# florianwechsung/alfi

Measured on AMD Instinct MI355X. Metric: V-cycles/sec on ldc3d P2-P0 (DoF*smooths/sec in dof_smooths_per_s), higher is better.
Workload: dtype f64

## Files before the change

alfi_amd/csrc/cond_layout.h:

```cpp
#pragma once
#include <cstdint>

#ifdef __HIPCC__
#define ALFI_HD __host__ __device__
#else
#define ALFI_HD
#endif

struct CondChunk {
  int64_t off;
  int64_t ubase;
  int64_t sidx0;
  int64_t stage_off;
  int32_t xq0, xq1;
  int32_t bq0, bq1;
  int32_t e0, ne;
  int32_t u0, nu;
  int32_t nI;
  int32_t xp0, bp0;
  int32_t pad;
};

#ifndef ALFI_COND_SIGMA_ROWS
#define ALFI_COND_SIGMA_ROWS 64
#endif
constexpr int COND_SIGMA_ROWS = ALFI_COND_SIGMA_ROWS;

constexpr int64_t COND_PER_PATCH_MIN = 1024;

ALFI_HD inline int cond_patch_waves(int max_pairs) {
#ifdef ALFI_COND_WAVES_FORCE
  (void)max_pairs;
  return ALFI_COND_WAVES_FORCE;
#else
  return max_pairs <= 64 ? 1 : max_pairs <= 128 ? 2 : max_pairs <= 256 ? 4 : 8;
#endif
}

ALFI_HD inline int cond_ldim(int rows) { return (rows + 1) & ~1; }
ALFI_HD inline int cond_pairs(int rows) { return (rows + 1) / 2; }
ALFI_HD inline int64_t cond_group_doubles(int m, int sc) {
  return (int64_t)cond_ldim(m) * m + (int64_t)cond_ldim(sc) * m + (int64_t)cond_ldim(m) * sc;
}
```

alfi_amd/csrc/kernels_bigpatch.hip:

```cpp
#include <algorithm>
#include <cstdlib>
#include <vector>
#include "common.h"
#include "row_piece.h"
#include "cond_apply.h"

constexpr int BIG_NB = 64;
constexpr int BIG_MAX_NP = PATCH_MAX;

template <int BS>
__global__ __launch_bounds__(256) void big_gather_kernel(int64_t p0, const int32_t* __restrict__ rowptr,
                                                          const int32_t* __restrict__ colidx,
                                                          const double* __restrict__ vals, int flat,
                                                          const int64_t* __restrict__ patch_ptr,
                                                          const int32_t* __restrict__ patch_dofs,
                                                          const int64_t* __restrict__ scr_ptr, double* __restrict__ scr) {
  __shared__ int32_t dofs_s[BIG_MAX_NP];
  const int64_t p = p0 + blockIdx.y;
  const int64_t off = patch_ptr[p];
  const int n = (int)(patch_ptr[p + 1] - off);
  const int N = (n + BIG_NB - 1) / BIG_NB * BIG_NB;
  double* S = scr + scr_ptr[blockIdx.y];
  for (int i = threadIdx.x; i < n; i += 256) dofs_s[i] = patch_dofs[off + i];
  const int chunk = (N + gridDim.x - 1) / gridDim.x;
// ... 683 lines not shown
  for (int k = 0; k < m; ++k) {
    double v = (lane >= k && lane < m) ? fabs(A[lane * m + k]) : -1.0;
    if (!(v == v)) v = INFINITY;
    int idx = lane;
#pragma unroll
    for (int o = 32; o > 0; o >>= 1) {
      const double ov = __shfl_xor(v, o);
      const int oi = __shfl_xor(idx, o);
      if (ov > v || (ov == v && oi < idx)) { v = ov; idx = oi; }
    }
    if (!(v > 0.0) || v == INFINITY) { bad = true; break; }
    if (lane == 0) perm[k] = idx;
    if (idx != k && lane < m) {
      const double t = A[k * m + lane];
      A[k * m + lane] = A[idx * m + lane];
      A[idx * m + lane] = t;
    }
    __syncthreads();
    const double ip = 1.0 / A[k * m + k];
    if (lane > k && lane < m) {
      const double l = A[lane * m + k] * ip;
      A[lane * m + k] = l;
      for (int j = k + 1; j < m; ++j) A[lane * m + j] = __builtin_fma(-l, A[k * m + j], A[lane * m + j]);
    }
    __syncthreads();
  }
  if (bad) {
    if (lane == 0) atomicExch(status, 1);
    return;
  }
  auto solve = [&](double* B, int nrhs, bool identity) {
    const bool act = lane < nrhs;
    for (int i = 0; i < m; ++i) Y[i * 64 + lane] = act ? (identity ? (i == lane ? 1.0 : 0.0) : B[(int64_t)lane * ldm + i]) : 0.0;
    for (int k = 0; k < m; ++k) {
      const int pk = perm[k];
      if (pk != k) {
        const double t = Y[k * 64 + lane];
        Y[k * 64 + lane] = Y[pk * 64 + lane];
        Y[pk * 64 + lane] = t;
      }
    }
    for (int i = 1; i < m; ++i) {
      double acc = Y[i * 64 + lane];
      for (int j = 0; j < i; ++j) acc = __builtin_fma(-A[i * m + j], Y[j * 64 + lane], acc);
      Y[i * 64 + lane] = acc;
    }
    for (int i = m - 1; i >= 0; --i) {
      double acc = Y[i * 64 + lane];
      for (int j = i + 1; j < m; ++j) acc = __builtin_fma(-A[i * m + j], Y[j * 64 + lane], acc);
      Y[i * 64 + lane] = acc / A[i * m + i];
    }
    if (act)
      for (int i = 0; i < m; ++i) B[(int64_t)lane * ldm + i] = Y[i * 64 + lane];
  };
  solve(W, sc, false);
  solve(X, m, true);
}

__global__ __launch_bounds__(256) void cond_schur_kernel(int64_t p0, CondDev cd, const int64_t* __restrict__ patch_ptr,
                                                          const int64_t* __restrict__ scr_ptr, double* __restrict__ scr) {
  const int64_t p = p0 + blockIdx.x;
  const int n = (int)(patch_ptr[p + 1] - patch_ptr[p]);
  const int s = n - cd.p_nI[p];
  const int N = (s + BIG_NB - 1) / BIG_NB * BIG_NB;
  double* S = scr + scr_ptr[blockIdx.x];
  for (int64_t g = cd.gptr[p]; g < cd.gptr[p + 1]; ++g) {
    const int m = cd.g_m[g], sc = cd.g_sc[g];
    const int ldm = cond_ldim(m), ldsc = cond_ldim(sc);
    const double* B = cd.mat + cd.g_mat[g] + (int64_t)ldm * m;
    const double* W = B + (int64_t)ldsc * m;
    const int32_t* si = cd.sidx + cd.g_sidx[g];
    for (int e = threadIdx.x; e < sc * sc; e += 256) {
      const int i = e % sc, j = e / sc;
      double acc = 0.0;
      for (int k = 0; k < m; ++k) acc = __builtin_fma(B[(int64_t)k * ldsc + i], W[(int64_t)j * ldm + k], acc);
      S[(int64_t)si[i] * N + si[j]] -= acc;
    }
    __syncthreads();
  }
}



template <bool NT, int COND_WAVES, int RU>
__global__ __launch_bounds__(64 * COND_WAVES) void cond_front_kernel(int64_t p0, int64_t p1, CondDev cd,
                                                                     const int64_t* __restrict__ patch_ptr,
                                                                     const int64_t* __restrict__ stage_ptr,
                                                                     const double* __restrict__ x, double* __restrict__ stage,
                                                                     int ordered) {
  extern __shared__ double cond_dsmem[];
  constexpr int NT_ = 64 * COND_WAVES;
  if (p0 + blockIdx.x >= p1) return;
  const int64_t p = ordered ? cd.order[blockIdx.x] : p0 + blockIdx.x;
  const int64_t off = patch_ptr[p];
  const int n = (int)(patch_ptr[p + 1] - off);
  const int nI = cd.p_nI[p];
  const int s = n - nI;
  const int64_t uo0 = cd.uptr[p];
  double* xs = cond_dsmem;
  double* ts = xs + n;
  double* us = ts + nI;
  for (int i0 = threadIdx.x; i0 < n; i0 += 4 * NT_) {
    int32_t d[4];
#pragma unroll
    for (int u = 0; u < 4; ++u) d[u] = (i0 + u * NT_ < n) ? cd.dofs[off + i0 + u * NT_] : 0;
    double v[4];
#pragma unroll
    for (int u = 0; u < 4; ++u) v[u] = (i0 + u * NT_ < n) ? x[d[u]] : 0.0;
#pragma unroll
    for (int u = 0; u < 4; ++u)
      if (i0 + u * NT_ < n) xs[i0 + u * NT_] = v[u];
  }
  __syncthreads();
  double* tmp = cd.tmp + off;
  const int64_t xp0 = cd.xp_ptr[p], bp0 = cd.bp_ptr[p];
  const int nxp = (int)(cd.xp_ptr[p + 1] - xp0), nbp = (int)(cd.bp_ptr[p + 1] - bp0);
  for (int q0 = 0; q0 < nxp; q0 += NT_) {
    const int q = q0 + threadIdx.x;
    const bool act = q < nxp;
    const int32_t g = act ? cd.xp_grp[xp0 + q] : (int32_t)cd.gptr[p];
    const int m = cd.g_m[g], o = cd.g_off[g], i = 2 * (q - cd.g_xp[g]);
    double t0 = 0.0, t1 = 0.0;
    cond_row2_dot<NT, RU>(cd.mat + cd.g_mat[g] + i, cond_ldim(m), act ? m : 0, xs + o, t0, t1);
    if (act) {
      ts[o + i] = t0;
      tmp[o + i] = t0;
      if (i + 1 < m) {
        ts[o + i + 1] = t1;
        tmp[o + i + 1] = t1;
      }
    }
  }
  __syncthreads();
  for (int q0 = 0; q0 < nbp; q0 += NT_) {
    const int q = q0 + threadIdx.x;
    const bool act = q < nbp;
    const int32_t g = act ? cd.bp_grp[bp0 + q] : (int32_t)cd.gptr[p];
    const int m = cd.g_m[g], sc = cd.g_sc[g], j = 2 * (q - cd.g_bp[g]);
    const int64_t ue = uo0 + cd.g_uoff[g] + j;
    const int32_t d0 = act ? cd.u_dst[ue] : 0, d1 = (act && j + 1 < sc) ? cd.u_dst[ue + 1] : 0;
    double u0 = 0.0, u1 = 0.0;
    cond_row2_dot<NT, RU>(cd.mat + cd.g_mat[g] + (int64_t)cond_ldim(m) * m + j, cond_ldim(sc), act ? m : 0,
                          ts + cd.g_off[g], u0, u1);
    if (act) {
      us[d0] = u0;
      if (j + 1 < sc) us[d1] = u1;
    }
  }
  __syncthreads();
  const int64_t srow0 = cd.sptr[p];
  const int32_t qb = cd.s_uptr[srow0];
  double* rhs = stage + stage_ptr[p] + nI;
  for (int i = threadIdx.x; i < s; i += NT_) {
    double acc = xs[nI + i];
    const int32_t qe = cd.s_uptr[srow0 + i + 1] - qb;
    for (int32_t q = cd.s_uptr[srow0 + i] - qb; q < qe; ++q) acc -= us[q];
    rhs[i] = acc;
  }
}

template <bool NT>
__global__ __launch_bounds__(256) void cond_sigma_kernel(int64_t c0, CondDev cd, const int64_t* __restrict__ patch_ptr,
                                                         const int64_t* __restrict__ stage_ptr,
                                                         const double* __restrict__ stage) {
  extern __shared__ double cond_dsmem[];
  const int64_t c = c0 + blockIdx.x;
  const int64_t p = cd.ch_patch[c];
  const int r0 = cd.ch_row[c];
  const int64_t off = patch_ptr[p];
  const int n = (int)(patch_ptr[p + 1] - off);
  const int nI = cd.p_nI[p];
  const int s = n - nI;
  const int ld = (s + 1) & ~1;
  const double* rhs = stage + stage_ptr[p] + nI;
  const int r1 = min(ld, r0 + COND_SIGMA_ROWS);
  const int share = (((r1 - r0) + 3) / 4 + 15) & ~15;
// ... 451 lines not shown
      hipLaunchKernelGGL(big_store_kernel, dim3(sx, (unsigned)nb), block, 0, ctx->stream, p0, d_patch_ptr, d_inv_ptr,
                         d_scr_ptr, result, inv);
    }
    e = hipGetLastError();
    if (e != hipSuccess) break;
  }
  if (e == hipSuccess) e = hipStreamSynchronize(ctx->stream);
  if (e != hipSuccess) return alfi_set_error(ctx, ALFI_E_HIP, "large-block factorisation failed: %s", hipGetErrorString(e));
  return 0;
}

int launch_big_factor_range(alfi_level* L, double* inv, int64_t p0, int64_t p1) {
  BigSource src;
  src.L = L;
  return big_factor_core(L->ctx, src, p0, p1, L->lay.patch_ptr.data(), L->patch_ptr, L->inv_ptr, inv, L->status);
}

int launch_big_factor_transfer(alfi_transfer* T) {
  BigSource src;
  src.T = T;
  std::vector<int64_t> hptr(T->nblk + 1);
  for (int64_t b = 0; b <= T->nblk; ++b) hptr[b] = b * T->m;
  return big_factor_core(T->ctx, src, 0, T->nblk, hptr.data(), T->pm_ptr, T->pm_inv_ptr, T->binv, T->status);
}

int launch_coarse_factor(alfi_level* L, double* out) {
  alfi_ctx* ctx = L->ctx;
  BigSource src;
  src.C = L;
  const int64_t hptr[2] = {0, L->n};
  int64_t* dptr = nullptr;
  ALFI_HIP_CHECK(ctx, hipMalloc((void**)&dptr, sizeof(hptr)));
  hipError_t e = hipMemcpy(dptr, hptr, sizeof(hptr), hipMemcpyHostToDevice);
  int rc = e == hipSuccess ? big_factor_core(ctx, src, 0, 1, hptr, dptr, nullptr, nullptr, L->status, out)
                           : alfi_set_error(ctx, ALFI_E_HIP, "hipMemcpy: %s", hipGetErrorString(e));
  (void)hipFree(dptr);
  if (rc == 0 && ctx->big_arena_bytes > ((size_t)1 << 30)) {
    (void)hipFree(ctx->big_arena);
    ctx->big_arena = nullptr;
    ctx->big_arena_bytes = 0;
  }
  return rc;
}

int launch_cond_factor(alfi_level* L) {
  BigSource src;
  src.K = L;
  return big_factor_core(L->ctx, src, 0, L->npatch, L->cplan.sptr.data(), L->cd.sptr, L->cd.sinv_ptr, L->cd.sinv, L->status);
}

int launch_cond_schur_one(alfi_level* L, int64_t p, const int64_t* d_zero, double* scr) {
  BigSource src;
  src.K = L;
  src.pivot_groups = true;
  src.fill(L->ctx, p, 1, d_zero, scr);
  ALFI_HIP_CHECK(L->ctx, hipGetLastError());
  return 0;
}

int launch_cond_apply_range(alfi_level* L, int64_t p0, int64_t p1, const double* x) {
  alfi_ctx* ctx = L->ctx;
  if (p1 <= p0) return 0;
  if (!L->cd.tmp) return alfi_set_error(ctx, ALFI_E_STATE, "condensed apply without its scratch (alfi_patches_set_groups)");
  dim3 grid((unsigned)(p1 - p0));
  const int ordered = p0 == 0 && p1 == L->npatch && L->cd.order ? 1 : 0;
  const int64_t c0 = L->cplan.chptr[p0], c1 = L->cplan.chptr[p1];
  if (p1 - p0 < COND_PER_PATCH_MIN) {
    const int64_t k0 = L->cplan.gcptr[p0], k1 = L->cplan.gcptr[p1];
    const size_t lds_f = (size_t)L->cplan.lds_gfront, lds_b = (size_t)L->cplan.lds_gback;
    const size_t lds_s = (size_t)(L->cplan.max_s + 2 + COND_SIGMA_ROWS) * sizeof(double);
    if (k1 > k0)
      hipLaunchKernelGGL((cond_gfront_kernel<false>), dim3((unsigned)(k1 - k0)), dim3(256), lds_f, ctx->stream, k0, L->cd, x);
    if (c1 > c0)
      hipLaunchKernelGGL((cond_gsigma_kernel<true>), dim3((unsigned)(c1 - c0)), dim3(256), lds_s, ctx->stream, c0, L->cd,
                         L->patch_ptr, L->stage_ptr, x, L->stage);
    if (k1 > k0)
      hipLaunchKernelGGL((cond_gback_kernel<false>), dim3((unsigned)(k1 - k0)), dim3(256), lds_b, ctx->stream, k0, L->cd,
                         L->stage);
    ALFI_HIP_CHECK(ctx, hipGetLastError());
    return 0;
  }
  const size_t lds_f = (size_t)L->cplan.lds_front, lds_s = (size_t)(L->cplan.max_s + 2) * sizeof(double);
  const size_t lds_b = (size_t)L->cplan.lds_back;
#define ALFI_COND_LAUNCH3(WV)                                                                                             \
  do {                                                                                                                    \
    if (lds_f > 64 * 1024)                                                                                                \
      ALFI_HIP_CHECK(ctx, hipFuncSetAttribute(reinterpret_cast<const void*>(&cond_front_kernel<false, WV, 8>),            \
                                              hipFuncAttributeMaxDynamicSharedMemorySize, (int)lds_f));                   \
    hipLaunchKernelGGL((cond_front_kernel<false, WV, 8>), dim3(grid.x), dim3(64 * WV), lds_f, ctx->stream, p0, p1, L->cd, \
                       L->patch_ptr, L->stage_ptr, x, L->stage, ordered);                                                 \
    if (c1 > c0)                                                                                                          \
      hipLaunchKernelGGL((cond_sigma_kernel<true>), dim3((unsigned)(c1 - c0)), dim3(256), lds_s, ctx->stream, c0, L->cd,  \
                         L->patch_ptr, L->stage_ptr, L->stage);                                                           \
    if (lds_b > 64 * 1024)                                                                                                \
      ALFI_HIP_CHECK(ctx, hipFuncSetAttribute(reinterpret_cast<const void*>(&cond_back_kernel<false, WV, 8>),             \
                                              hipFuncAttributeMaxDynamicSharedMemorySize, (int)lds_b));                   \
    hipLaunchKernelGGL((cond_back_kernel<false, WV, 8>), dim3(grid.x), dim3(64 * WV), lds_b, ctx->stream, p0, p1, L->cd,  \
                       L->patch_ptr, L->stage_ptr, L->stage, ordered);                                                    \
  } while (0)
#ifdef ALFI_COND_WAVES_FORCE
  ALFI_COND_LAUNCH3(ALFI_COND_WAVES_FORCE);
#else
  switch (cond_patch_waves(L->cplan.max_pairs)) {
    case 1: ALFI_COND_LAUNCH3(1); break;
    case 2: ALFI_COND_LAUNCH3(2); break;
    case 4: ALFI_COND_LAUNCH3(4); break;
    default: ALFI_COND_LAUNCH3(8); break;
  }
#endif
#undef ALFI_COND_LAUNCH3
  ALFI_HIP_CHECK(ctx, hipGetLastError());
  return 0;
}

#include "mf_coarse.h"
```

alfi_amd/csrc/patch_plan.h:

```cpp
#pragma once
#include <algorithm>
#include <climits>
#include <cstdarg>
#include <cstdint>
#include <cstdio>
#include <string>
#include <vector>
#include "cond_layout.h"

#pragma GCC visibility push(hidden)

constexpr int PLAN_E_ARG = -2;
constexpr int SMALL_PATCH_MAX = 160;
constexpr int PATCH_MAX = 4096;
constexpr int COND_LDS_MAX_BYTES = 150 * 1024;
constexpr int COND_GROUP_MAX = 64;
constexpr int COND_CHUNK_PAIRS = 256;
constexpr int MULT_WAVE_NODES = 64;

inline int plan_fail(std::string* err, const char* fmt, ...) {
  char buf[1024];
  va_list ap;
  va_start(ap, fmt);
  vsnprintf(buf, sizeof(buf), fmt, ap);
// ... 67 lines not shown
  out->stage_ptr = std::move(stage_ptr);
  out->dof_ptr = std::move(dof_ptr);
  out->dof_pos = std::move(dof_pos);
  out->sum_n = sum_n;
  out->sum_n2 = sum_n2;
  out->max_np = max_np;
  out->inv_doubles = ip;
  out->stage_len = sp;
  return 0;
}

ALFI_HD inline int64_t piece_index(int r, int c, int n, int ld, int min_rows) {
  int row0 = r & ~127, rows = 128;
  if (row0 + 128 > ld) {
    const int rem = ld - row0;
    int rr = r - row0;
    for (int bit = 64; bit >= min_rows; bit >>= 1) {
      if (rem & bit) {
        if (rr < bit) {
          rows = bit;
          break;
        }
        rr -= bit;
        row0 += bit;
      }
    }
  }
  return (int64_t)row0 * n + (int64_t)c * rows + (r - row0);
}
ALFI_HD inline int64_t patch_inv_index(int r, int c, int n, int ld) { return piece_index(r, c, n, ld, 2); }

constexpr int F32_ROWS = 4;
constexpr int F32_ALIGN = 32;

ALFI_HD inline int f32_ld(int n) { return (n + F32_ROWS - 1) & ~(F32_ROWS - 1); }
ALFI_HD inline int64_t f32_patch_floats(int n) { return ((int64_t)n * f32_ld(n) + F32_ALIGN - 1) & ~(int64_t)(F32_ALIGN - 1); }
ALFI_HD inline int64_t f32_inv_index(int r, int c, int n) { return piece_index(r, c, n, f32_ld(n), F32_ROWS); }
inline int64_t plan_f32_offsets(int64_t npatch, const int64_t* pptr, std::vector<int64_t>* f32_ptr) {
  f32_ptr->resize((size_t)npatch + 1);
  int64_t ip = 0;
  for (int64_t p = 0; p < npatch; ++p) {
    (*f32_ptr)[(size_t)p] = ip;
    ip += f32_patch_floats((int)(pptr[p + 1] - pptr[p]));
  }
  (*f32_ptr)[(size_t)npatch] = ip;
  return ip;
}
inline int64_t plan_f32_ranges(int64_t npatch, const int64_t* inv_ptr, int64_t cap, std::vector<int64_t>* ranges) {
  ranges->assign(1, 0);
  int64_t work = 0;
  for (int64_t p0 = 0; p0 < npatch;) {
    int64_t p1 = p0 + 1;
    while (p1 < npatch && inv_ptr[p1 + 1] - inv_ptr[p0] <= cap) ++p1;
    work = std::max(work, inv_ptr[p1] - inv_ptr[p0]);
    ranges->push_back(p1);
    p0 = p1;
  }
  return work;
}

inline int big_split(int64_t npatch, int max_np) {
  const int64_t want = (2048 + npatch - 1) / npatch;
  const int pieces = (max_np + 127) / 128;
  const int cap = (pieces + 3) / 4;
  return (int)(want < 1 ? 1 : (want > cap ? cap : want));
}

struct CondPlan {
  std::vector<int32_t> dofs, slot;
  std::vector<int64_t> gptr, g_mat, g_sidx;
  std::vector<int32_t> g_off, g_m, g_sc, g_uoff, g_xp, g_bp;
  std::vector<int32_t> sidx;
  std::vector<int32_t> p_nI, order;
  std::vector<int64_t> sptr, sinv_ptr, uptr, xp_ptr, bp_ptr;
  std::vector<int32_t> s_uptr, s_uidx, u_dst;
  std::vector<int64_t> chptr, gcptr;
  std::vector<int32_t> ch_patch, ch_row, xp_grp, bp_grp;
  std::vector<CondChunk> gc;
  int64_t ngroups = 0, mat_doubles = 0, sinv_doubles = 0;
  int lds_bytes = 0, lds_front = 0, lds_back = 0, lds_gfront = 0, lds_gback = 0;
  int max_s = 0;
  int max_m = 0;
  int max_pairs = 0;
  int umax = 0;

  void release_tables() {
    CondPlan keep;
    keep.sptr.swap(sptr); keep.gptr.swap(gptr); keep.chptr.swap(chptr); keep.gcptr.swap(gcptr);
    keep.ngroups = ngroups; keep.mat_doubles = mat_doubles; keep.sinv_doubles = sinv_doubles;
    keep.lds_bytes = lds_bytes; keep.lds_front = lds_front; keep.lds_back = lds_back;
    keep.lds_gfront = lds_gfront; keep.lds_gback = lds_gback;
    keep.max_s = max_s; keep.max_m = max_m; keep.max_pairs = max_pairs; keep.umax = umax;
    *this = std::move(keep);
  }
};

inline int plan_condensed(int bs, int64_t nb, int64_t npatch, const int64_t* pp, const int32_t* pd, const int32_t* group,
                          const int32_t* rowptr, const int32_t* colidx, int sigma_rows, CondPlan* out, std::string* err) {
  const int64_t sum_n = pp[npatch];
  std::vector<int32_t> c_dofs(sum_n), c_slot(sum_n), g_off, g_m, g_sc, g_uoff, sidx, p_nI(npatch), s_uptr, s_uidx;
  std::vector<int64_t> gptr(npatch + 1, 0), g_mat, g_sidx, sptr(npatch + 1, 0), sinv_ptr(npatch + 1, 0);
  std::vector<int32_t> node_pos(nb, -1);
  int64_t mat_off = 0, sinv_off = 0;
  int lds_max = 0, umax = 0, smax = 0;
  s_uptr.push_back(0);
  for (int64_t p = 0; p < npatch; ++p) {
    const int64_t off = pp[p];
    const int n = (int)(pp[p + 1] - off);
    if (n % bs != 0) return plan_fail(err, "patch %lld: condensed factors need patches of whole nodes", (long long)p);
    const int nn = n / bs;
    std::vector<int32_t> lab(nn);
    bool one_label = patch_of_whole_nodes(bs, pd + off, n);
    for (int i = 0; i < nn; ++i) {
      lab[i] = group[off + (int64_t)i * bs];
      for (int c = 0; c < bs; ++c)
        if (group[off + (int64_t)i * bs + c] != lab[i]) one_label = false;
    }
    if (!one_label)
      return plan_fail(err, "patch %lld: entries of a node must be adjacent and carry one group label", (long long)p);
    std::vector<int32_t> labels;
    for (int i = 0; i < nn; ++i) if (lab[i] >= 0) labels.push_back(lab[i]);
    std::sort(labels.begin(), labels.end());
    labels.erase(std::unique(labels.begin(), labels.end()), labels.end());
    const int ng = (int)labels.size();
    std::vector<int32_t> order;
    order.reserve(nn);
    std::vector<int32_t> gstart(ng + 1, 0);
    for (int g = 0; g < ng; ++g) {
      for (int i = 0; i < nn; ++i) if (lab[i] == labels[g]) order.push_back(i);
      gstart[g + 1] = (int32_t)order.size();
    }
    const int nIn = (int)order.size();
    for (int i = 0; i < nn; ++i) if (lab[i] < 0) order.push_back(i);
    for (int q = 0; q < nn; ++q) {
      node_pos[pd[off + (int64_t)order[q] * bs] / bs] = q;
      for (int c = 0; c < bs; ++c) {
        c_dofs[off + (int64_t)q * bs + c] = pd[off + (int64_t)order[q] * bs + c];
        c_slot[off + (int64_t)q * bs + c] = order[q] * bs + c;
      }
    }
    const int sn = nn - nIn, s = sn * bs;
    p_nI[p] = nIn * bs;
    sptr[p + 1] = sptr[p] + s;
    const int64_t ld_s = (s + 1) & ~1;
    sinv_ptr[p] = sinv_off;
    sinv_off += ((int64_t)s * ld_s + 15) & ~(int64_t)15;
    if (s > smax) smax = s;
    gptr[p + 1] = gptr[p] + ng;
    std::vector<std::vector<int32_t>> row_contrib(sn);
    int uoff = 0;
    std::vector<char> mark(sn);
    for (int g = 0; g < ng; ++g) {
      std::fill(mark.begin(), mark.end(), 0);
      for (int q = gstart[g]; q < gstart[g + 1]; ++q) {
        const int node = pd[off + (int64_t)order[q] * bs] / bs;
        for (int32_t k = rowptr[node]; k < rowptr[node + 1]; ++k) {
          const int cq = node_pos[colidx[k] & 0x7fffffff];
          if (cq < 0) continue;
          if (cq >= nIn) mark[cq - nIn] = 1;
          else if (cq < gstart[g] || cq >= gstart[g + 1])
            return plan_fail(err, "patch %lld: groups %d and another one are coupled by an operator entry "
                             "(a group may touch the rest of the patch only through unlabelled dofs)", (long long)p, labels[g]);
        }
      }
      const int m = (gstart[g + 1] - gstart[g]) * bs;
      int scn = 0;
      g_sidx.push_back((int64_t)sidx.size());
      for (int j = 0; j < sn; ++j)
        if (mark[j]) {
          for (int c = 0; c < bs; ++c) sidx.push_back(j * bs + c);
          row_contrib[j].push_back(uoff + scn * bs);
          ++scn;
        }
      const int sc = scn * bs;
      if (m > COND_GROUP_MAX || sc > COND_GROUP_MAX)
        return plan_fail(err, "patch %lld: group %d holds %d entries coupled to %d skeleton entries; the "
                         "condensed factors handle at most 64 of each", (long long)p, labels[g], m, sc);
      g_off.push_back(gstart[g] * bs);
      g_m.push_back(m);
      g_sc.push_back(sc);
      g_uoff.push_back(uoff);
      g_mat.push_back(mat_off);
      mat_off += cond_group_doubles(m, sc);
      uoff += sc;
    }
    if (uoff > umax) umax = uoff;
    for (int j = 0; j < sn; ++j)
      for (int c = 0; c < bs; ++c) {
        for (int32_t u : row_contrib[j]) s_uidx.push_back(u + c);
        s_uptr.push_back((int32_t)s_uidx.size());
      }
    for (int i = 0; i < nn; ++i) node_pos[pd[off + (int64_t)i * bs] / bs] = -1;
    const int lds = (n + uoff + s + 2) * (int)sizeof(double);
    if (lds > lds_max) lds_max = lds;
  }
  sinv_ptr[npatch] = sinv_off;
  if (lds_max > COND_LDS_MAX_BYTES) return plan_fail(err, "condensed apply would need %d bytes of LDS per patch", lds_max);
  if (g_off.empty()) return plan_fail(err, "no group label >= 0: nothing to condense");
  if (sidx.empty()) sidx.push_back(0);
  if (s_uidx.empty()) s_uidx.push_back(0);
  std::vector<int32_t> order((size_t)npatch);
  {
    std::vector<int64_t> pbytes((size_t)npatch, 0);
    for (int64_t p = 0; p < npatch; ++p) {
      const int64_t s = sptr[p + 1] - sptr[p];
      pbytes[p] = s * s;
      for (int64_t g = gptr[p]; g < gptr[p + 1]; ++g) pbytes[p] += cond_group_doubles(g_m[g], g_sc[g]);
    }
    for (int64_t p = 0; p < npatch; ++p) order[p] = (int32_t)p;
    std::stable_sort(order.begin(), order.end(), [&](int32_t a, int32_t b) { return pbytes[a] > pbytes[b]; });
  }
  std::vector<int32_t> ch_patch, ch_row, xp_grp, bp_grp, g_xp(g_m.size()), g_bp(g_m.size()), u_dst;
  std::vector<int64_t> chptr((size_t)npatch + 1, 0), uptr((size_t)npatch + 1, 0), xp_ptr((size_t)npatch + 1, 0),
      bp_ptr((size_t)npatch + 1, 0);
  int lds_front = 0, lds_back = 0, max_pairs = 0;
  for (int64_t p = 0; p < npatch; ++p) {
    const int s = (int)(sptr[p + 1] - sptr[p]), ld = (s + 1) & ~1;
    for (int r = 0; r < ld; r += sigma_rows) {
      ch_patch.push_back((int32_t)p);
      ch_row.push_back(r);
    }
    chptr[p + 1] = (int64_t)ch_patch.size();
    int uo = 0, xp = 0, bp = 0;
    for (int64_t g = gptr[p]; g < gptr[p + 1]; ++g) {
      g_xp[g] = xp;
      g_bp[g] = bp;
      for (int i = 0; i < cond_pairs(g_m[g]); ++i) xp_grp.push_back((int32_t)g);
      for (int j = 0; j < cond_pairs(g_sc[g]); ++j) bp_grp.push_back((int32_t)g);
      xp += cond_pairs(g_m[g]);
      bp += cond_pairs(g_sc[g]);
      uo += g_sc[g];
    }
    uptr[p + 1] = uptr[p] + uo;
    xp_ptr[p + 1] = xp_ptr[p] + xp;
    bp_ptr[p + 1] = bp_ptr[p] + bp;
    const int32_t qb = s_uptr[sptr[p]], qe = s_uptr[sptr[p + 1]];
    if (qe - qb != uo) return plan_fail(err, "patch %lld: inconsistent skeleton contributions", (long long)p);
    u_dst.resize((size_t)uptr[p + 1]);
    for (int32_t q = qb; q < qe; ++q) u_dst[uptr[p] + s_uidx[q]] = q - qb;
    max_pairs = std::max(max_pairs, std::max(xp, bp));
    lds_front = std::max(lds_front, (int)((pp[p + 1] - pp[p] + p_nI[p] + uo + 2) * (int64_t)sizeof(double)));
    lds_back = std::max(lds_back, (int)((s + uo + 2) * (int64_t)sizeof(double)));
  }
  if (ch_patch.empty()) { ch_patch.push_back(0); ch_row.push_back(0); }
  if (xp_grp.empty()) xp_grp.push_back(0);
  if (bp_grp.empty()) bp_grp.push_back(0);
  if (u_dst.empty()) u_dst.push_back(0);
  if (lds_front > COND_LDS_MAX_BYTES) return plan_fail(err, "condensed apply would need %d bytes of LDS per patch", lds_front);
  std::vector<CondChunk> gc;
  std::vector<int64_t> gcptr((size_t)npatch + 1, 0), stage_off((size_t)npatch + 1, 0);
  for (int64_t p = 0; p < npatch; ++p)
    stage_off[p + 1] = stage_off[p] + ((pp[p + 1] - pp[p] + 1) & ~(int64_t)1);
  int lds_gf = 0, lds_gb = 0;
  for (int64_t p = 0; p < npatch; ++p) {
    int64_t g = gptr[p];
    while (g < gptr[p + 1]) {
      CondChunk c;
      const int64_t ga = g;
      int xp = 0, bp = 0, ne = 0, nu = 0;
      while (g < gptr[p + 1] && xp + cond_pairs(g_m[g]) <= COND_CHUNK_PAIRS && bp + cond_pairs(g_sc[g]) <= COND_CHUNK_PAIRS) {
        xp += cond_pairs(g_m[g]);
        bp += cond_pairs(g_sc[g]);
        ne += g_m[g];
        nu += g_sc[g];
        ++g;
      }
      c.off = pp[p]; c.ubase = uptr[p]; c.sidx0 = g_sidx[ga]; c.stage_off = stage_off[p];
      c.xq0 = (int32_t)(xp_ptr[p] + g_xp[ga]); c.xq1 = c.xq0 + xp;
      c.bq0 = (int32_t)(bp_ptr[p] + g_bp[ga]); c.bq1 = c.bq0 + bp;
      c.e0 = g_off[ga]; c.ne = ne; c.u0 = g_uoff[ga]; c.nu = nu; c.nI = p_nI[p]; c.pad = 0;
      c.xp0 = (int32_t)xp_ptr[p]; c.bp0 = (int32_t)bp_ptr[p];
      gc.push_back(c);
      lds_gf = std::max(lds_gf, (int)(2 * ne * sizeof(double)));
      lds_gb = std::max(lds_gb, (int)(nu * sizeof(double)));
    }
    gcptr[p + 1] = (int64_t)gc.size();
  }
  if (xp_ptr[npatch] > INT32_MAX || bp_ptr[npatch] > INT32_MAX)
    return plan_fail(err, "condensed factors: too many row pairs on one level");
  if (gc.empty()) gc.push_back(CondChunk());
  CondPlan& o = *out;
  o.ngroups = (int64_t)g_off.size();
  o.mat_doubles = mat_off;
  o.sinv_doubles = sinv_off;
  o.lds_bytes = lds_max;
  o.lds_front = lds_front;
  o.lds_back = lds_back;
  o.lds_gfront = lds_gf + 16;
  o.lds_gback = lds_gb + 16;
  o.max_s = smax;
  o.max_m = g_m.empty() ? 0 : *std::max_element(g_m.begin(), g_m.end());
  o.max_pairs = max_pairs;
  o.umax = umax;
  o.dofs = std::move(c_dofs); o.slot = std::move(c_slot);
  o.gptr = std::move(gptr); o.g_mat = std::move(g_mat); o.g_sidx = std::move(g_sidx);
  o.g_off = std::move(g_off); o.g_m = std::move(g_m); o.g_sc = std::move(g_sc); o.g_uoff = std::move(g_uoff);
  o.g_xp = std::move(g_xp); o.g_bp = std::move(g_bp);
  o.sidx = std::move(sidx);
  o.p_nI = std::move(p_nI); o.order = std::move(order);
  o.sptr = std::move(sptr); o.sinv_ptr = std::move(sinv_ptr); o.uptr = std::move(uptr);
  o.xp_ptr = std::move(xp_ptr); o.bp_ptr = std::move(bp_ptr);
  o.s_uptr = std::move(s_uptr); o.s_uidx = std::move(s_uidx); o.u_dst = std::move(u_dst);
  o.chptr = std::move(chptr); o.gcptr = std::move(gcptr);
  o.ch_patch = std::move(ch_patch); o.ch_row = std::move(ch_row); o.xp_grp = std::move(xp_grp); o.bp_grp = std::move(bp_grp);
  o.gc = std::move(gc);
  return 0;
}

struct SweepPlan {
  bool big = false;
  std::vector<int32_t> seq;
  std::vector<int64_t> wave_ptr;
  std::vector<int32_t> items, pred0, succ_ptr, succ;
  int32_t nitems = 0;
  std::vector<int32_t> rowtab;
};

inline int check_sweep(int bs, int64_t npatch, const int64_t* pp, const int32_t* pd, int small_max, int64_t nit,
                       const int64_t* iterset, bool* big, std::string* err) {
  *big = false;
  for (int64_t p = 0; p < npatch; ++p) {
    const int64_t a = pp[p], b = pp[p + 1];
    if (b - a > small_max || (b - a) / bs > MULT_WAVE_NODES) *big = true;
    if ((b - a) % bs != 0) return plan_fail(err, "patch %lld: multiplicative sweeps need patches of whole nodes", (long long)p);
    if (!patch_of_whole_nodes(bs, pd + a, b - a)) return plan_fail(err, "patch %lld does not consist of whole nodes", (long long)p);
  }
  for (int64_t t = 0; t < nit; ++t)
    if (iterset[t] < 0 || iterset[t] >= npatch) return plan_fail(err, "iteration set entry out of range");
  return 0;
}

inline int plan_sweep(int bs, int64_t nb, int64_t npatch, const int64_t* pp, const int32_t* pd, const int32_t* rowptr,
                      const int32_t* colidx, int64_t nit, const int64_t* iterset, bool symmetrise, bool big, SweepPlan* out,
                      std::string* err) {
  out->big = big;
  std::vector<int32_t> node_wave(nb, -1), wave_of(nit);
  int32_t nwave = 0;
  for (int64_t t = 0; t < nit; ++t) {
    const int64_t p = iterset[t];
    const int64_t a = pp[p], b = pp[p + 1];
    int32_t w = -1;
    for (int64_t q = a; q < b; q += bs) {
      const int32_t node = pd[q] / bs;
      for (int32_t k = rowptr[node]; k < rowptr[node + 1]; ++k) {
        const int32_t c = colidx[k] & 0x7fffffff;
        if (node_wave[c] > w) w = node_wave[c];
      }
    }
    ++w;
    wave_of[t] = w;
    if (w + 1 > nwave) nwave = w + 1;
    for (int64_t q = a; q < b; q += bs) node_wave[pd[q] / bs] = w;
  }
  std::vector<int64_t>& wave_ptr = out->wave_ptr;
  wave_ptr.assign(nwave + 1, 0);
  for (int64_t t = 0; t < nit; ++t) wave_ptr[wave_of[t] + 1]++;
  for (int32_t w = 0; w < nwave; ++w) wave_ptr[w + 1] += wave_ptr[w];
  std::vector<int32_t>& seq = out->seq;
  seq.resize(nit);
  {
    std::vector<int64_t> fill(wave_ptr.begin(), wave_ptr.end() - 1);
    for (int64_t t = 0; t < nit; ++t) seq[fill[wave_of[t]]++] = (int32_t)iterset[t];
  }
  if (!big) {
    std::vector<int32_t>& rowtab = out->rowtab;
    rowtab.assign((size_t)npatch * MULT_WAVE_NODES * 3, 0);
    for (int64_t p = 0; p < npatch; ++p) {
      const int64_t a = pp[p], b = pp[p + 1];
      for (int64_t q = a, i = 0; q < b; q += bs, ++i) {
        const int32_t node = pd[q] / bs;
        int32_t* rt = &rowtab[((size_t)p * MULT_WAVE_NODES + (size_t)i) * 3];
        rt[0] = rowptr[node];
        rt[1] = rowptr[node + 1] - rowptr[node];
        rt[2] = node;
      }
// ... 50 lines not shown
```

Measured before the change: 8.431.

## Add latency-hiding front kernel splitting x-pair and b-pair waves for small groups

Adds a specialised condensed-apply front path for groups with at most 16 rows. Each thread issues its matrix-row loads for both the interior solve and the Schur coupling before the x gather completes. Dedicated waves handle the x-pairs and b-pairs separately, so the dependent loads overlap and the serialized per-pair loops are removed. The cost is larger blocks, extra register pressure from holding 16 double2 values per thread, and a new code path that is chosen at plan time.

After: 8.672 (median of 6 runs). 1.03x the previous value.

```diff
diff --git a/alfi_amd/csrc/cond_layout.h b/alfi_amd/csrc/cond_layout.h
--- a/alfi_amd/csrc/cond_layout.h
+++ b/alfi_amd/csrc/cond_layout.h
@@ -37,6 +37,15 @@
 #endif
 }
 
+#ifndef ALFI_COND_AHEAD
+#define ALFI_COND_AHEAD 1
+#endif
+constexpr int COND_AHEAD_M = 16;
+ALFI_HD inline bool cond_ahead(int max_m, int max_pairs) {
+  return ALFI_COND_AHEAD != 0 && max_m <= COND_AHEAD_M && max_pairs <= 64 * cond_patch_waves(max_pairs);
+}
+ALFI_HD inline int cond_ahead_front_waves(int xpairs, int bpairs) { return (xpairs + 63) / 64 + (bpairs + 63) / 64; }
+
 ALFI_HD inline int cond_ldim(int rows) { return (rows + 1) & ~1; }
 ALFI_HD inline int cond_pairs(int rows) { return (rows + 1) / 2; }
 ALFI_HD inline int64_t cond_group_doubles(int m, int sc) {
diff --git a/alfi_amd/csrc/kernels_bigpatch.hip b/alfi_amd/csrc/kernels_bigpatch.hip
--- a/alfi_amd/csrc/kernels_bigpatch.hip
+++ b/alfi_amd/csrc/kernels_bigpatch.hip
@@ -789,8 +789,127 @@
 
 
 
-template <bool NT, int COND_WAVES, int RU>
-__global__ __launch_bounds__(64 * COND_WAVES) void cond_front_kernel(int64_t p0, int64_t p1, CondDev cd,
+template <bool NT, int A>
+__device__ __forceinline__ void cond_row2_request(const double* __restrict__ M, int ld, int kn, big_d2 (&a)[A]) {
+#pragma unroll
+  for (int u = 0; u < A; ++u) {
+    const big_d2* q = reinterpret_cast<const big_d2*>(M + (int64_t)u * ld);
+    const big_d2 z = {0.0, 0.0};
+    a[u] = (u < kn) ? (NT ? __builtin_nontemporal_load(q) : *q) : z;
+  }
+}
+template <int A>
+__device__ __forceinline__ void cond_row2_sum(const big_d2 (&a)[A], int kn, const double* __restrict__ v, double& acc0,
+                                              double& acc1) {
+#pragma unroll
+  for (int u = 0; u < A; ++u) {
+    const double vk = (u < kn) ? v[u] : 0.0;
+    acc0 = __builtin_fma(a[u].x, vk, acc0);
+    acc1 = __builtin_fma(a[u].y, vk, acc1);
+  }
+}
+
+template <typename T>
+__device__ __forceinline__ void cond_arrived(T& v) {
+  asm volatile("" : "+v"(v));
+}
+
+template <bool NT>
+__device__ __forceinline__ void cond_front_ahead(int64_t p, const CondDev& cd, const int64_t* __restrict__ patch_ptr,
+                                                 const int64_t* __restrict__ stage_ptr, const double* __restrict__ x,
+                                                 double* __restrict__ stage, double* __restrict__ smem) {
+  const int NT_ = (int)blockDim.x, tid = (int)threadIdx.x;
+  const int64_t off = patch_ptr[p];
+  const int n = (int)(patch_ptr[p + 1] - off);
+  const int nI = cd.p_nI[p];
+  const int s = n - nI;
+  const int64_t uo0 = cd.uptr[p];
+  const int64_t xp0 = cd.xp_ptr[p], bp0 = cd.bp_ptr[p];
+  const int nxp = (int)(cd.xp_ptr[p + 1] - xp0), nbp = (int)(cd.bp_ptr[p + 1] - bp0);
+  const int64_t srow0 = cd.sptr[p];
+  double* rhs = stage + stage_ptr[p] + nI;
+  double* xs = smem;
+  double* ts = xs + n;
+  double* us = ts + nI;
+  double* tmp = cd.tmp + off;
+  const int xw = (nxp + 63) >> 6;
+  const bool isx = (tid >> 6) < xw;
+  const int q = isx ? tid : tid - 64 * xw;
+  const bool act = isx ? q < nxp : q < nbp;
+  const bool bact = act && !isx;
+  int32_t d[4];
+#pragma unroll
+  for (int u = 0; u < 4; ++u) d[u] = (tid + u * NT_ < n) ? cd.dofs[off + tid + u * NT_] : 0;
+  const int32_t* pgrp = isx ? cd.xp_grp + xp0 : cd.bp_grp + bp0;
+  int32_t g = act ? pgrp[q] : 0;
+  const int32_t qb = cd.s_uptr[srow0];
+  const int32_t su0 = tid < s ? cd.s_uptr[srow0 + tid] : 0, su1 = tid < s ? cd.s_uptr[srow0 + tid + 1] : 0;
+#pragma unroll
+  for (int u = 0; u < 4; ++u) cond_arrived(d[u]);
+  cond_arrived(g);
+  double v[4];
+#pragma unroll
+  for (int u = 0; u < 4; ++u) v[u] = (tid + u * NT_ < n) ? x[d[u]] : 0.0;
+  int32_t m = act ? cd.g_m[g] : 0, o = act ? cd.g_off[g] : 0;
+  const int32_t* g_pr = isx ? cd.g_xp : cd.g_bp;
+  int32_t pr = act ? g_pr[g] : 0;
+  int64_t mat = act ? cd.g_mat[g] : 0;
+  int32_t sc = bact ? cd.g_sc[g] : 0, uoff = bact ? cd.g_uoff[g] : 0;
+  cond_arrived(m);
+  cond_arrived(o);
+  cond_arrived(pr);
+  cond_arrived(mat);
+  cond_arrived(sc);
+  cond_arrived(uoff);
+  const int r = 2 * (q - pr);
+  const int ld = isx ? cond_ldim(m) : cond_ldim(sc);
+  const double* M = cd.mat + mat + (isx ? 0 : (int64_t)cond_ldim(m) * m) + r;
+  const int64_t ue = uo0 + uoff + r;
+  big_d2 a[COND_AHEAD_M];
+  cond_row2_request<NT, COND_AHEAD_M>(M, ld, m, a);
+  const int32_t d0 = bact ? cd.u_dst[ue] : 0, d1 = (bact && r + 1 < sc) ? cd.u_dst[ue + 1] : 0;
+#pragma unroll
+  for (int u = 0; u < 4; ++u)
+    if (tid + u * NT_ < n) xs[tid + u * NT_] = v[u];
+  for (int i = tid + 4 * NT_; i < n; i += NT_) xs[i] = x[cd.dofs[off + i]];
+  __syncthreads();
+  if (isx) {
+    double t0 = 0.0, t1 = 0.0;
+    cond_row2_sum<COND_AHEAD_M>(a, m, xs + o, t0, t1);
+    if (act) {
+      ts[o + r] = t0;
+      tmp[o + r] = t0;
+      if (r + 1 < m) {
+        ts[o + r + 1] = t1;
+        tmp[o + r + 1] = t1;
+      }
+    }
+  }
+  __syncthreads();
+  if (!isx) {
+    double u0 = 0.0, u1 = 0.0;
+    cond_row2_sum<COND_AHEAD_M>(a, m, ts + o, u0, u1);
+    if (act) {
+      us[d0] = u0;
+      if (r + 1 < sc) us[d1] = u1;
+    }
+  }
+  __syncthreads();
+  if (tid < s) {
+    double acc = xs[nI + tid];
+    for (int32_t k = su0 - qb; k < su1 - qb; ++k) acc -= us[k];
+    rhs[tid] = acc;
+  }
+  for (int i = tid + NT_; i < s; i += NT_) {
+    double acc = xs[nI + i];
+    const int32_t qe = cd.s_uptr[srow0 + i + 1] - qb;
+    for (int32_t k = cd.s_uptr[srow0 + i] - qb; k < qe; ++k) acc -= us[k];
+    rhs[i] = acc;
+  }
+}
+
+template <bool NT, int COND_WAVES, int RU, bool AHEAD = false>
+__global__ __launch_bounds__(64 * COND_WAVES * (AHEAD ? 2 : 1)) void cond_front_kernel(int64_t p0, int64_t p1, CondDev cd,
                                                                      const int64_t* __restrict__ patch_ptr,
                                                                      const int64_t* __restrict__ stage_ptr,
                                                                      const double* __restrict__ x, double* __restrict__ stage,
@@ -799,6 +918,10 @@
   constexpr int NT_ = 64 * COND_WAVES;
   if (p0 + blockIdx.x >= p1) return;
   const int64_t p = ordered ? cd.order[blockIdx.x] : p0 + blockIdx.x;
+  if constexpr (AHEAD) {
+    cond_front_ahead<NT>(p, cd, patch_ptr, stage_ptr, x, stage, cond_dsmem);
+    return;
+  }
   const int64_t off = patch_ptr[p];
   const int n = (int)(patch_ptr[p + 1] - off);
   const int nI = cd.p_nI[p];
@@ -1416,13 +1539,13 @@
   }
   const size_t lds_f = (size_t)L->cplan.lds_front, lds_s = (size_t)(L->cplan.max_s + 2) * sizeof(double);
   const size_t lds_b = (size_t)L->cplan.lds_back;
-#define ALFI_COND_LAUNCH3(WV)                                                                                             \
+#define ALFI_COND_LAUNCH3(WV, AH, FW)                                                                                     \
   do {                                                                                                                    \
     if (lds_f > 64 * 1024)                                                                                                \
-      ALFI_HIP_CHECK(ctx, hipFuncSetAttribute(reinterpret_cast<const void*>(&cond_front_kernel<false, WV, 8>),            \
+      ALFI_HIP_CHECK(ctx, hipFuncSetAttribute(reinterpret_cast<const void*>(&cond_front_kernel<false, WV, 8, AH>),        \
                                               hipFuncAttributeMaxDynamicSharedMemorySize, (int)lds_f));                   \
-    hipLaunchKernelGGL((cond_front_kernel<false, WV, 8>), dim3(grid.x), dim3(64 * WV), lds_f, ctx->stream, p0, p1, L->cd, \
-                       L->patch_ptr, L->stage_ptr, x, L->stage, ordered);                                                 \
+    hipLaunchKernelGGL((cond_front_kernel<false, WV, 8, AH>), dim3(grid.x), dim3(64 * (FW)), lds_f, ctx->stream, p0, p1,  \
+                       L->cd, L->patch_ptr, L->stage_ptr, x, L->stage, ordered);                                          \
     if (c1 > c0)                                                                                                          \
       hipLaunchKernelGGL((cond_sigma_kernel<true>), dim3((unsigned)(c1 - c0)), dim3(256), lds_s, ctx->stream, c0, L->cd,  \
                          L->patch_ptr, L->stage_ptr, L->stage);                                                           \
@@ -1432,16 +1555,29 @@
     hipLaunchKernelGGL((cond_back_kernel<false, WV, 8>), dim3(grid.x), dim3(64 * WV), lds_b, ctx->stream, p0, p1, L->cd,  \
                        L->patch_ptr, L->stage_ptr, L->stage, ordered);                                                    \
   } while (0)
+#if ALFI_COND_AHEAD
+#define ALFI_COND_LAUNCH3_W(WV)                                  \
+  do {                                                           \
+    if (ahead)                                                   \
+      ALFI_COND_LAUNCH3(WV, true, L->cplan.front_waves);         \
+    else                                                         \
+      ALFI_COND_LAUNCH3(WV, false, WV);                          \
+  } while (0)
+  const bool ahead = cond_ahead(L->cplan.max_m, L->cplan.max_pairs);
+#else
+#define ALFI_COND_LAUNCH3_W(WV) ALFI_COND_LAUNCH3(WV, false, WV)
+#endif
 #ifdef ALFI_COND_WAVES_FORCE
-  ALFI_COND_LAUNCH3(ALFI_COND_WAVES_FORCE);
+  ALFI_COND_LAUNCH3_W(ALFI_COND_WAVES_FORCE);
 #else
   switch (cond_patch_waves(L->cplan.max_pairs)) {
-    case 1: ALFI_COND_LAUNCH3(1); break;
-    case 2: ALFI_COND_LAUNCH3(2); break;
-    case 4: ALFI_COND_LAUNCH3(4); break;
-    default: ALFI_COND_LAUNCH3(8); break;
+    case 1: ALFI_COND_LAUNCH3_W(1); break;
+    case 2: ALFI_COND_LAUNCH3_W(2); break;
+    case 4: ALFI_COND_LAUNCH3_W(4); break;
+    default: ALFI_COND_LAUNCH3_W(8); break;
   }
 #endif
+#undef ALFI_COND_LAUNCH3_W
 #undef ALFI_COND_LAUNCH3
   ALFI_HIP_CHECK(ctx, hipGetLastError());
   return 0;
diff --git a/alfi_amd/csrc/patch_plan.h b/alfi_amd/csrc/patch_plan.h
--- a/alfi_amd/csrc/patch_plan.h
+++ b/alfi_amd/csrc/patch_plan.h
@@ -173,6 +173,7 @@
   int max_s = 0;
   int max_m = 0;
   int max_pairs = 0;
+  int front_waves = 1;
   int umax = 0;
 
   void release_tables() {
@@ -181,7 +182,7 @@
     keep.ngroups = ngroups; keep.mat_doubles = mat_doubles; keep.sinv_doubles = sinv_doubles;
     keep.lds_bytes = lds_bytes; keep.lds_front = lds_front; keep.lds_back = lds_back;
     keep.lds_gfront = lds_gfront; keep.lds_gback = lds_gback;
-    keep.max_s = max_s; keep.max_m = max_m; keep.max_pairs = max_pairs; keep.umax = umax;
+    keep.max_s = max_s; keep.max_m = max_m; keep.max_pairs = max_pairs; keep.front_waves = front_waves; keep.umax = umax;
     *this = std::move(keep);
   }
 };
@@ -304,7 +305,7 @@
   std::vector<int32_t> ch_patch, ch_row, xp_grp, bp_grp, g_xp(g_m.size()), g_bp(g_m.size()), u_dst;
   std::vector<int64_t> chptr((size_t)npatch + 1, 0), uptr((size_t)npatch + 1, 0), xp_ptr((size_t)npatch + 1, 0),
       bp_ptr((size_t)npatch + 1, 0);
-  int lds_front = 0, lds_back = 0, max_pairs = 0;
+  int lds_front = 0, lds_back = 0, max_pairs = 0, front_waves = 1;
   for (int64_t p = 0; p < npatch; ++p) {
     const int s = (int)(sptr[p + 1] - sptr[p]), ld = (s + 1) & ~1;
     for (int r = 0; r < ld; r += sigma_rows) {
@@ -330,6 +331,7 @@
     u_dst.resize((size_t)uptr[p + 1]);
     for (int32_t q = qb; q < qe; ++q) u_dst[uptr[p] + s_uidx[q]] = q - qb;
     max_pairs = std::max(max_pairs, std::max(xp, bp));
+    front_waves = std::max(front_waves, cond_ahead_front_waves(xp, bp));
     lds_front = std::max(lds_front, (int)((pp[p + 1] - pp[p] + p_nI[p] + uo + 2) * (int64_t)sizeof(double)));
     lds_back = std::max(lds_back, (int)((s + uo + 2) * (int64_t)sizeof(double)));
   }
@@ -382,6 +384,7 @@
   o.max_s = smax;
   o.max_m = g_m.empty() ? 0 : *std::max_element(g_m.begin(), g_m.end());
   o.max_pairs = max_pairs;
+  o.front_waves = front_waves;
   o.umax = umax;
   o.dofs = std::move(c_dofs); o.slot = std::move(c_slot);
   o.gptr = std::move(gptr); o.g_mat = std::move(g_mat); o.g_sidx = std::move(g_sidx);
```
